# kivicode/TensorHive-Fixed

Measured on AMD Instinct MI355X. Metric: llama3_8b_bf16_ddp_train_tokens_per_sec, higher is better.
Workload: dtype bf16; 1 GPU; model=Llama-3-8B, global_batch=8, micro_batch=8, grad_accum=1, seq_len=4096, parallelism=dp1, optimizer=AdamW (fp32 master, fused flat kernel, clip 1.0), zero=0, attention=hip, gemm_table=True, gemm_table_kind=gemm_gfx950_t32768.csv

## Files before the change

tensorhive_fixed_amd/ops/csrc/cross_entropy.hip:

```cpp
#include "th_common.h"

__global__ __launch_bounds__(512) void ce_fwd_bwd_kernel(ushort* __restrict__ logits, long ld,
                                                         const long* __restrict__ target,
                                                         float* __restrict__ loss,
                                                         float* __restrict__ lse_out, int V,
                                                         float grad_scale, int ignore_index) {
  __shared__ float sm[16], ss[16];
  const long row = blockIdx.x;
  ushort* lr = logits + row * ld;
  const int nvec = (ld & 7) == 0 ? (V >> 3) : 0;
  float m = -INFINITY, s = 0.f;
  for (int i = threadIdx.x; i < nvec; i += blockDim.x) {
    const ushort8 x = reinterpret_cast<const ushort8*>(lr)[i];
    float vmax = -INFINITY;
    float f[8];
#pragma unroll
    for (int j = 0; j < 8; ++j) {
      f[j] = bf2f(x[j]);
      vmax = fmaxf(vmax, f[j]);
    }
    float vs = 0.f;
#pragma unroll
    for (int j = 0; j < 8; ++j) vs += __expf(f[j] - vmax);
    lse_merge(m, s, vmax, vs);
  }
  for (int i = (nvec << 3) + threadIdx.x; i < V; i += blockDim.x) lse_merge(m, s, bf2f(lr[i]), 1.f);
#pragma unroll
  for (int o = 32; o > 0; o >>= 1) {
    const float m2 = __shfl_xor(m, o, 64), s2 = __shfl_xor(s, o, 64);
    lse_merge(m, s, m2, s2);
  }
  const int lane = threadIdx.x & 63, wid = threadIdx.x >> 6;
  if (lane == 0) { sm[wid] = m; ss[wid] = s; }
  __syncthreads();
  m = sm[0]; s = ss[0];
  for (int w = 1; w < (int)(blockDim.x >> 6); ++w) lse_merge(m, s, sm[w], ss[w]);
  const float lse = m + __logf(s);
  const long tgt = target[row];
  const bool valid = tgt != ignore_index && tgt >= 0 && tgt < V;
  if (threadIdx.x == 0) {
    lse_out[row] = lse;
    loss[row] = valid ? (lse - bf2f(lr[tgt])) : 0.f;
  }
  __syncthreads();
  const float gs = valid ? grad_scale : 0.f;
  for (int i = threadIdx.x; i < nvec; i += blockDim.x) {
    const ushort8 x = reinterpret_cast<const ushort8*>(lr)[i];
    ushort8 o;
#pragma unroll
    for (int j = 0; j < 8; ++j) {
      float p = __expf(bf2f(x[j]) - lse);
      if (valid && (long)(i * 8 + j) == tgt) p -= 1.f;
      o[j] = f2bf(p * gs);
    }
    reinterpret_cast<ushort8*>(lr)[i] = o;
  }
  for (int i = (nvec << 3) + threadIdx.x; i < V; i += blockDim.x) {
    float p = __expf(bf2f(lr[i]) - lse);
    if (valid && (long)i == tgt) p -= 1.f;
    lr[i] = f2bf(p * gs);
  }
}

extern "C" int th_ce_fwd_bwd(void* logits, long ld, const long* target, float* loss, float* lse,
                             long rows, int V, float grad_scale, int ignore_index, hipStream_t s) {
  if (rows <= 0 || V <= 0 || ld < V) return -1;
  ce_fwd_bwd_kernel<<<(unsigned)rows, 512, 0, s>>>((ushort*)logits, ld, target, loss, lse, V,
                                                  grad_scale, ignore_index);
  TH_CHECK_LAUNCH();
}
```

tensorhive_fixed_amd/ops/csrc/rmsnorm.hip:

```cpp
#include "th_common.h"

template <int MAXV, bool ADD>
__global__ __launch_bounds__(256) void rmsnorm_fwd_kernel(const ushort* __restrict__ x,
                                                              const ushort* __restrict__ addend,
                                                              ushort* __restrict__ xsum,
                                                              const ushort* __restrict__ w,
                                                              ushort* __restrict__ y,
                                                              float* __restrict__ rstd_out, int D,
                                                              float eps) {
  __shared__ float red[16];
  const int row = blockIdx.x;
  const int nvec = D >> 3;
  const ushort8* xr = reinterpret_cast<const ushort8*>(x + (size_t)row * D);
  ushort8 cache[MAXV];
  float ss = 0.f;
#pragma unroll
  for (int i = 0; i < MAXV; ++i) {
    const int v = threadIdx.x + i * blockDim.x;
    if (v < nvec) {
      cache[i] = xr[v];
      if (ADD) {
        const ushort8 a = reinterpret_cast<const ushort8*>(addend + (size_t)row * D)[v];
#pragma unroll
        for (int j = 0; j < 8; ++j) cache[i][j] = f2bf(bf2f(cache[i][j]) + bf2f(a[j]));
        reinterpret_cast<ushort8*>(xsum + (size_t)row * D)[v] = cache[i];
      }
#pragma unroll
      for (int j = 0; j < 8; ++j) {
        const float f = bf2f(cache[i][j]);
        ss += f * f;
      }
    }
  }
  ss = block_sum(ss, red);
  const float r = rsqrtf(ss / (float)D + eps);
  if (threadIdx.x == 0) rstd_out[row] = r;
  const ushort8* wr = reinterpret_cast<const ushort8*>(w);
  ushort8* yr = reinterpret_cast<ushort8*>(y + (size_t)row * D);
#pragma unroll
  for (int i = 0; i < MAXV; ++i) {
    const int v = threadIdx.x + i * blockDim.x;
    if (v < nvec) {
      const ushort8 wv = wr[v];
      ushort8 o;
#pragma unroll
      for (int j = 0; j < 8; ++j) o[j] = f2bf(bf2f(cache[i][j]) * r * bf2f(wv[j]));
      yr[v] = o;
    }
  }
}

template <int MAXV>
__global__ __launch_bounds__(256) void rmsnorm_bwd_kernel(const ushort* __restrict__ dy,
                                                          const ushort* __restrict__ x,
                                                          const ushort* __restrict__ w,
                                                          const float* __restrict__ rstd,
                                                          ushort* __restrict__ dx,
                                                          float* __restrict__ ws, int T, int D,
                                                          const ushort* __restrict__ dres) {
  __shared__ float red[16];
  const int nvec = D >> 3;
  float dwacc[MAXV][8];
  float wreg[MAXV][8];
  const ushort8* wr = reinterpret_cast<const ushort8*>(w);
#pragma unroll
  for (int i = 0; i < MAXV; ++i) {
    const int v = threadIdx.x + i * blockDim.x;
    ushort8 wv = (v < nvec) ? wr[v] : ushort8(0);
#pragma unroll
    for (int j = 0; j < 8; ++j) {
      dwacc[i][j] = 0.f;
      wreg[i][j] = bf2f(wv[j]);
    }
  }
  for (int row = blockIdx.x; row < T; row += gridDim.x) {
    const ushort8* xr = reinterpret_cast<const ushort8*>(x + (size_t)row * D);
    const ushort8* gr = reinterpret_cast<const ushort8*>(dy + (size_t)row * D);
    ushort8 xc[MAXV], gc[MAXV], rc[MAXV];
    float dot = 0.f;
#pragma unroll
    for (int i = 0; i < MAXV; ++i) {
      const int v = threadIdx.x + i * blockDim.x;
      if (v < nvec) {
        xc[i] = xr[v];
        gc[i] = gr[v];
        rc[i] = dres ? reinterpret_cast<const ushort8*>(dres + (size_t)row * D)[v] : ushort8(0);
#pragma unroll
        for (int j = 0; j < 8; ++j) dot += bf2f(gc[i][j]) * wreg[i][j] * bf2f(xc[i][j]);
      }
    }
    dot = block_sum(dot, red);
    const float r = rstd[row];
    const float c = dot * r * r * r / (float)D;
    ushort8* dxr = reinterpret_cast<ushort8*>(dx + (size_t)row * D);
#pragma unroll
    for (int i = 0; i < MAXV; ++i) {
      const int v = threadIdx.x + i * blockDim.x;
      if (v < nvec) {
        ushort8 o;
#pragma unroll
        for (int j = 0; j < 8; ++j) {
          const float xf = bf2f(xc[i][j]), gf = bf2f(gc[i][j]);
          o[j] = f2bf(r * gf * wreg[i][j] - xf * c + bf2f(rc[i][j]));
          dwacc[i][j] += gf * xf * r;
        }
        dxr[v] = o;
      }
    }
  }
  float* wsr = ws + (size_t)blockIdx.x * D;
#pragma unroll
  for (int i = 0; i < MAXV; ++i) {
    const int v = threadIdx.x + i * blockDim.x;
    if (v < nvec) {
      float4v* p = reinterpret_cast<float4v*>(wsr + v * 8);
      p[0] = float4v{dwacc[i][0], dwacc[i][1], dwacc[i][2], dwacc[i][3]};
      p[1] = float4v{dwacc[i][4], dwacc[i][5], dwacc[i][6], dwacc[i][7]};
    }
  }
}

__global__ __launch_bounds__(256) void slab_reduce_bf16_kernel(const float* __restrict__ ws, ushort* __restrict__ out,
                                                               int nslab, int D, int accumulate) {
  __shared__ float4v part[16][16];
  const int cg = threadIdx.x & 15, sg = threadIdx.x >> 4;
  const int c = blockIdx.x * 64 + cg * 4;
  float4v acc = {0.f, 0.f, 0.f, 0.f};
  if (c < D) {
#pragma unroll 4
    for (int b = sg; b < nslab; b += 16) acc += *reinterpret_cast<const float4v*>(ws + (size_t)b * D + c);
  }
  part[sg][cg] = acc;
  __syncthreads();
  if (sg == 0 && c < D) {
    float4v t = part[0][cg];
#pragma unroll
    for (int k = 1; k < 16; ++k) t += part[k][cg];
#pragma unroll
    for (int j = 0; j < 4; ++j) {
      float v = t[j];
      if (accumulate) v += bf2f(out[c + j]);
      out[c + j] = f2bf(v);
    }
  }
}

static int pick_maxv(int D, int threads) { return (D / 8 + threads - 1) / threads; }

extern "C" int th_rmsnorm_fwd(const void* x, const void* w, void* y, float* rstd, int T, int D,
                              float eps, hipStream_t s) {
  if (D % 8 != 0 || T <= 0) return -1;
  const int mv = pick_maxv(D, 256);
  dim3 g(T), b(256);
  if (mv <= 2)
    rmsnorm_fwd_kernel<2, false><<<g, b, 0, s>>>((const ushort*)x, nullptr, nullptr, (const ushort*)w, (ushort*)y, rstd, D, eps);
  else if (mv <= 4)
    rmsnorm_fwd_kernel<4, false><<<g, b, 0, s>>>((const ushort*)x, nullptr, nullptr, (const ushort*)w, (ushort*)y, rstd, D, eps);
  else if (mv <= 8)
    rmsnorm_fwd_kernel<8, false><<<g, b, 0, s>>>((const ushort*)x, nullptr, nullptr, (const ushort*)w, (ushort*)y, rstd, D, eps);
  else
    return -2;
  TH_CHECK_LAUNCH();
}

extern "C" int th_rmsnorm_add_fwd(const void* x, const void* addend, const void* w, void* xsum, void* y,
                                  float* rstd, int T, int D, float eps, hipStream_t s) {
  if (D % 8 != 0 || T <= 0) return -1;
  const int mv = pick_maxv(D, 256);
  dim3 g(T), b(256);
#define TH_RMS_ADD(MV)                                                                                   \
  rmsnorm_fwd_kernel<MV, true><<<g, b, 0, s>>>((const ushort*)x, (const ushort*)addend, (ushort*)xsum, \
                                               (const ushort*)w, (ushort*)y, rstd, D, eps)
  if (mv <= 2)
    TH_RMS_ADD(2);
  else if (mv <= 4)
    TH_RMS_ADD(4);
  else if (mv <= 8)
    TH_RMS_ADD(8);
  else
    return -2;
#undef TH_RMS_ADD
  TH_CHECK_LAUNCH();
}

extern "C" int th_rmsnorm_bwd(const void* dy, const void* x, const void* w, const float* rstd,
                              void* dx, void* dw, float* ws, int nblk, int T, int D,
                              int accumulate, const void* dres, hipStream_t s) {
  if (D % 8 != 0 || T <= 0 || nblk <= 0) return -1;
  const int mv = pick_maxv(D, 256);
  dim3 g(nblk), b(256);
  if (mv <= 2)
    rmsnorm_bwd_kernel<2><<<g, b, 0, s>>>((const ushort*)dy, (const ushort*)x, (const ushort*)w, rstd, (ushort*)dx, ws, T, D, (const ushort*)dres);
  else if (mv <= 4)
    rmsnorm_bwd_kernel<4><<<g, b, 0, s>>>((const ushort*)dy, (const ushort*)x, (const ushort*)w, rstd, (ushort*)dx, ws, T, D, (const ushort*)dres);
  else if (mv <= 8)
    rmsnorm_bwd_kernel<8><<<g, b, 0, s>>>((const ushort*)dy, (const ushort*)x, (const ushort*)w, rstd, (ushort*)dx, ws, T, D, (const ushort*)dres);
  else
    return -2;
  slab_reduce_bf16_kernel<<<dim3((D + 63) / 64), dim3(256), 0, s>>>(ws, (ushort*)dw, nblk, D, accumulate);
  TH_CHECK_LAUNCH();
}
```

tensorhive_fixed_amd/ops/csrc/swiglu.hip:

```cpp
#include "th_common.h"

__device__ __forceinline__ float sigmoidf_(float g) { return 1.f / (1.f + __expf(-g)); }

__global__ __launch_bounds__(256) void swiglu_fwd_kernel(const ushort* __restrict__ gu,
                                                         ushort* __restrict__ out, long T, int F) {
  const int cpr = F >> 3;
  for (long row = blockIdx.x; row < T; row += gridDim.x) {
    const ushort* g_row = gu + row * 2 * F;
    ushort* o_row = out + row * F;
    for (int c = threadIdx.x; c < cpr; c += blockDim.x) {
      const ushort8 g = *reinterpret_cast<const ushort8*>(g_row + c * 8);
      const ushort8 u = *reinterpret_cast<const ushort8*>(g_row + F + c * 8);
      ushort8 o;
#pragma unroll
      for (int j = 0; j < 8; ++j) {
        const float gf = bf2f(g[j]);
        o[j] = f2bf(gf * sigmoidf_(gf) * bf2f(u[j]));
      }
      *reinterpret_cast<ushort8*>(o_row + c * 8) = o;
    }
  }
}

__global__ __launch_bounds__(256) void swiglu_bwd_kernel(const ushort* __restrict__ dout,
                                                         const ushort* __restrict__ gu,
                                                         ushort* __restrict__ dgu, long T, int F) {
  const int cpr = F >> 3;
  for (long row = blockIdx.x; row < T; row += gridDim.x) {
    for (int c = threadIdx.x; c < cpr; c += blockDim.x) {
      const ushort8 g = *reinterpret_cast<const ushort8*>(gu + row * 2 * F + c * 8);
      const ushort8 u = *reinterpret_cast<const ushort8*>(gu + row * 2 * F + F + c * 8);
      const ushort8 d = *reinterpret_cast<const ushort8*>(dout + row * F + c * 8);
      ushort8 dg, du;
#pragma unroll
      for (int j = 0; j < 8; ++j) {
        const float gf = bf2f(g[j]), uf = bf2f(u[j]), df = bf2f(d[j]);
        const float sg = sigmoidf_(gf);
        const float silu = gf * sg;
        du[j] = f2bf(df * silu);
        dg[j] = f2bf(df * uf * sg * (1.f + gf * (1.f - sg)));
      }
      *reinterpret_cast<ushort8*>(dgu + row * 2 * F + c * 8) = dg;
      *reinterpret_cast<ushort8*>(dgu + row * 2 * F + F + c * 8) = du;
    }
  }
}

constexpr int ST_R = 128, ST_C = 64;

__device__ __forceinline__ int st_swz(int r) { return 2 * (((r >> 1) & 1) | (((r >> 3) & 1) << 1)); }
__device__ __forceinline__ int st_off(int r, int chunk) { return r * 128 + ((chunk ^ st_swz(r)) << 4); }

typedef short i16x4s __attribute__((ext_vector_type(4)));
#define ST_LDS __attribute__((address_space(3)))

__global__ __launch_bounds__(256) void swiglu_bwd_t_kernel(const ushort* __restrict__ dout,
                                                           const ushort* __restrict__ gu,
                                                           ushort* __restrict__ dgu,
                                                           ushort* __restrict__ dguT, long T, int F) {
  __shared__ __attribute__((aligned(16))) char tile[2 * ST_R * 128];
  const int tid = threadIdx.x;
  const long ntc = F / ST_C;
  const long r0 = (blockIdx.x / ntc) * ST_R, c0 = (blockIdx.x % ntc) * ST_C;
  const int lch = tid & 7, lc = lch * 8;
  ushort8 g[4], u[4], d[4];
#pragma unroll
  for (int i = 0; i < 4; ++i) {
    const long row = r0 + (tid >> 3) + 32 * i;
    const long rr = row < T ? row : T - 1;
    g[i] = *reinterpret_cast<const ushort8*>(gu + rr * 2 * F + c0 + lc);
    u[i] = *reinterpret_cast<const ushort8*>(gu + rr * 2 * F + F + c0 + lc);
    d[i] = *reinterpret_cast<const ushort8*>(dout + rr * F + c0 + lc);
  }
#pragma unroll
  for (int i = 0; i < 4; ++i) {
    const int lr = (tid >> 3) + 32 * i;
    const long row = r0 + lr;
    ushort8 dg, du;
#pragma unroll
    for (int j = 0; j < 8; ++j) {
      const float gf = bf2f(g[i][j]), uf = bf2f(u[i][j]), df = bf2f(d[i][j]);
      const float sg = sigmoidf_(gf);
      du[j] = f2bf(df * gf * sg);
      dg[j] = f2bf(df * uf * sg * (1.f + gf * (1.f - sg)));
    }
    if (row < T) {
      *reinterpret_cast<ushort8*>(dgu + row * 2 * F + c0 + lc) = dg;
      *reinterpret_cast<ushort8*>(dgu + row * 2 * F + F + c0 + lc) = du;
    }
    *reinterpret_cast<ushort8*>(tile + st_off(lr, lch)) = dg;
    *reinterpret_cast<ushort8*>(tile + ST_R * 128 + st_off(lr, lch)) = du;
  }
  __syncthreads();
  const int lane = tid & 63, w = tid >> 6, grp = lane >> 4, i16 = lane & 15, q = i16 >> 2, p = i16 & 3;
#pragma unroll
  for (int k = 0; k < 8; ++k) {
    const int step = w * 8 + k;
    const int half = step >> 4, fb = (step >> 2) & 3, tg0 = (step & 3) * 32;
    const int rbase = tg0 + 8 * grp;
    const int col = fb * 16 + 4 * p;
    const char* base = tile + half * ST_R * 128 + ((col & 7) << 1);
    const int ch = col >> 3;
    const i16x4s lo = __builtin_amdgcn_ds_read_tr16_b64_v4i16((ST_LDS i16x4s*)(base + st_off(rbase + q, ch)));
    const i16x4s hi = __builtin_amdgcn_ds_read_tr16_b64_v4i16((ST_LDS i16x4s*)(base + st_off(rbase + 4 + q, ch)));
    ushort8 o;
#pragma unroll
    for (int e = 0; e < 4; ++e) {
      o[e] = (ushort)lo[e];
      o[4 + e] = (ushort)hi[e];
    }
    const long feat = (long)half * F + c0 + fb * 16 + i16;
    const long tok = r0 + rbase;
    if (tok < T) *reinterpret_cast<ushort8*>(dguT + feat * T + tok) = o;
  }
}

static unsigned grid_for(long rows) {
  long g = rows;
  if (g > 4096) g = 4096;
  if (g < 1) g = 1;
  return (unsigned)g;
}

extern "C" int th_swiglu_fwd(const void* gu, void* out, long T, int F, hipStream_t s) {
  if (F % 8 != 0 || T <= 0) return -1;
  swiglu_fwd_kernel<<<grid_for(T), 256, 0, s>>>((const ushort*)gu, (ushort*)out, T, F);
  TH_CHECK_LAUNCH();
}

extern "C" int th_swiglu_bwd(const void* dout, const void* gu, void* dgu, long T, int F,
                             hipStream_t s) {
  if (F % 8 != 0 || T <= 0) return -1;
  swiglu_bwd_kernel<<<grid_for(T), 256, 0, s>>>((const ushort*)dout, (const ushort*)gu,
                                                          (ushort*)dgu, T, F);
  TH_CHECK_LAUNCH();
}

extern "C" int th_swiglu_bwd_t(const void* dout, const void* gu, void* dgu, void* dguT, long T, int F,
                               hipStream_t s) {
  if (F % ST_C != 0 || T <= 0 || T % 8 != 0) return -1;
  const long tiles = ((T + ST_R - 1) / ST_R) * (F / ST_C);
  if (tiles > 0x7fffffffL) return -2;
  swiglu_bwd_t_kernel<<<(unsigned)tiles, 256, 0, s>>>((const ushort*)dout, (const ushort*)gu, (ushort*)dgu,
                                                      (ushort*)dguT, T, F);
  TH_CHECK_LAUNCH();
}
```

tensorhive_fixed_amd/ops/csrc/transpose.hip:

```cpp
#include "th_common.h"

template <int TR, int TC>
__global__ __launch_bounds__(256) void transpose_bf16_kernel(const ushort* __restrict__ in,
                                                             ushort* __restrict__ out, long R, long C,
                                                             long ld_in) {
  constexpr int PITCH = TC + 2;
  constexpr int LPR = TC / 8;
  constexpr int RPP = 256 / LPR;
  constexpr int OPL = 256 / TC;
  constexpr int RPL = TR / OPL;
  __shared__ ushort tile[TR * PITCH];
  const int tid = threadIdx.x;
  const long ntc = (C + TC - 1) / TC;
  const long bt = blockIdx.x;
  const long r0 = (bt / ntc) * TR, c0 = (bt % ntc) * TC;

  const int lc = (tid % LPR) * 8;
  ushort8 v[TR / RPP];
#pragma unroll
  for (int i = 0; i < TR / RPP; ++i) {
    const int lr = tid / LPR + RPP * i;
    v[i] = ushort8(0);
    if (r0 + lr < R && c0 + lc < C) v[i] = *reinterpret_cast<const ushort8*>(in + (r0 + lr) * ld_in + c0 + lc);
  }
#pragma unroll
  for (int i = 0; i < TR / RPP; ++i) {
    const int lr = tid / LPR + RPP * i;
    unsigned* dst = reinterpret_cast<unsigned*>(tile + lr * PITCH + lc);
#pragma unroll
    for (int j = 0; j < 4; ++j) dst[j] = (unsigned)v[i][2 * j] | ((unsigned)v[i][2 * j + 1] << 16);
  }
  __syncthreads();

  const int oc = tid / OPL;
  const int orr = (tid % OPL) * RPL;
  if (c0 + oc >= C) return;
  ushort* orow = out + (c0 + oc) * R + r0 + orr;
#pragma unroll
  for (int q = 0; q < RPL / 8; ++q) {
    ushort8 w;
#pragma unroll
    for (int j = 0; j < 8; ++j) w[j] = tile[(orr + 8 * q + j) * PITCH + oc];
    if (r0 + orr + 8 * q < R) *reinterpret_cast<ushort8*>(orow + 8 * q) = w;
  }
}

extern "C" int th_transpose_bf16(const void* in, void* out, long R, long C, long ld_in, int tile, hipStream_t s) {
  if (R <= 0 || C <= 0 || R % 8 || C % 8 || ld_in % 8 || ld_in < C) return -1;
  auto launch = [&](auto kern, long tr, long tc) {
    const long tiles = ((R + tr - 1) / tr) * ((C + tc - 1) / tc);
    if (tiles > 0x7fffffffL) return -2;
    kern<<<(unsigned)tiles, 256, 0, s>>>((const ushort*)in, (ushort*)out, R, C, ld_in);
    return (int)hipGetLastError();
  };
  if (tile == 0) tile = C > 16384 ? 1 : 3;
  switch (tile) {
    case 2: return launch(transpose_bf16_kernel<128, 128>, 128, 128);
    case 3: return launch(transpose_bf16_kernel<64, 128>, 64, 128);
    default: return launch(transpose_bf16_kernel<128, 64>, 128, 64);
  }
}
```

Before: 27020 tokens/s.

## Batch loads in CE, SwiGLU, RMSNorm bwd and use LDS transpose reads

The cross-entropy kernel now keeps the whole logits row in registers, so the gradient pass no longer reloads it from memory. RMSNorm backward prefetches the next row's inputs while the current row is computed. SwiGLU kernels batch eight vector loads per thread and use nontemporal loads and stores. The transpose kernel switches to a swizzled LDS layout read with ds_read_tr16_b64 transposing loads. Together these aim to cut memory traffic and latency stalls, at the cost of higher register pressure and lower occupancy.

```diff
diff --git a/tensorhive_fixed_amd/ops/csrc/cross_entropy.hip b/tensorhive_fixed_amd/ops/csrc/cross_entropy.hip
--- a/tensorhive_fixed_amd/ops/csrc/cross_entropy.hip
+++ b/tensorhive_fixed_amd/ops/csrc/cross_entropy.hip
@@ -1,5 +1,8 @@
 #include "th_common.h"
 
+constexpr int CE_SLOTS = 32;
+
+template <bool HOLD>
 __global__ __launch_bounds__(512) void ce_fwd_bwd_kernel(ushort* __restrict__ logits, long ld,
                                                          const long* __restrict__ target,
                                                          float* __restrict__ loss,
@@ -10,8 +13,8 @@
   ushort* lr = logits + row * ld;
   const int nvec = (ld & 7) == 0 ? (V >> 3) : 0;
   float m = -INFINITY, s = 0.f;
-  for (int i = threadIdx.x; i < nvec; i += blockDim.x) {
-    const ushort8 x = reinterpret_cast<const ushort8*>(lr)[i];
+  ushort8 held[HOLD ? CE_SLOTS : 1];
+  auto merge_vec = [&](const ushort8 x) {
     float vmax = -INFINITY;
     float f[8];
 #pragma unroll
@@ -23,6 +26,18 @@
 #pragma unroll
     for (int j = 0; j < 8; ++j) vs += __expf(f[j] - vmax);
     lse_merge(m, s, vmax, vs);
+  };
+  if (HOLD) {
+#pragma unroll
+    for (int k = 0; k < CE_SLOTS; ++k) {
+      const int i = threadIdx.x + k * 512;
+      if (i < nvec) held[k] = reinterpret_cast<const ushort8*>(lr)[i];
+    }
+#pragma unroll
+    for (int k = 0; k < CE_SLOTS; ++k)
+      if ((int)threadIdx.x + k * 512 < nvec) merge_vec(held[k]);
+  } else {
+    for (int i = threadIdx.x; i < nvec; i += blockDim.x) merge_vec(reinterpret_cast<const ushort8*>(lr)[i]);
   }
   for (int i = (nvec << 3) + threadIdx.x; i < V; i += blockDim.x) lse_merge(m, s, bf2f(lr[i]), 1.f);
 #pragma unroll
@@ -44,8 +59,7 @@
   }
   __syncthreads();
   const float gs = valid ? grad_scale : 0.f;
-  for (int i = threadIdx.x; i < nvec; i += blockDim.x) {
-    const ushort8 x = reinterpret_cast<const ushort8*>(lr)[i];
+  auto grad_vec = [&](const ushort8 x, int i) {
     ushort8 o;
 #pragma unroll
     for (int j = 0; j < 8; ++j) {
@@ -54,6 +68,15 @@
       o[j] = f2bf(p * gs);
     }
     reinterpret_cast<ushort8*>(lr)[i] = o;
+  };
+  if (HOLD) {
+#pragma unroll
+    for (int k = 0; k < CE_SLOTS; ++k) {
+      const int i = threadIdx.x + k * 512;
+      if (i < nvec) grad_vec(held[k], i);
+    }
+  } else {
+    for (int i = threadIdx.x; i < nvec; i += blockDim.x) grad_vec(reinterpret_cast<const ushort8*>(lr)[i], i);
   }
   for (int i = (nvec << 3) + threadIdx.x; i < V; i += blockDim.x) {
     float p = __expf(bf2f(lr[i]) - lse);
@@ -65,7 +88,12 @@
 extern "C" int th_ce_fwd_bwd(void* logits, long ld, const long* target, float* loss, float* lse,
                              long rows, int V, float grad_scale, int ignore_index, hipStream_t s) {
   if (rows <= 0 || V <= 0 || ld < V) return -1;
-  ce_fwd_bwd_kernel<<<(unsigned)rows, 512, 0, s>>>((ushort*)logits, ld, target, loss, lse, V,
-                                                  grad_scale, ignore_index);
+  const bool hold = (ld & 7) == 0 && ((uintptr_t)logits & 15) == 0 && (V >> 3) <= 512 * CE_SLOTS;
+  if (hold)
+    ce_fwd_bwd_kernel<true><<<(unsigned)rows, 512, 0, s>>>((ushort*)logits, ld, target, loss, lse, V,
+                                                          grad_scale, ignore_index);
+  else
+    ce_fwd_bwd_kernel<false><<<(unsigned)rows, 512, 0, s>>>((ushort*)logits, ld, target, loss, lse, V,
+                                                           grad_scale, ignore_index);
   TH_CHECK_LAUNCH();
 }
diff --git a/tensorhive_fixed_amd/ops/csrc/rmsnorm.hip b/tensorhive_fixed_amd/ops/csrc/rmsnorm.hip
--- a/tensorhive_fixed_amd/ops/csrc/rmsnorm.hip
+++ b/tensorhive_fixed_amd/ops/csrc/rmsnorm.hip
@@ -73,24 +73,39 @@
       wreg[i][j] = bf2f(wv[j]);
     }
   }
-  for (int row = blockIdx.x; row < T; row += gridDim.x) {
+  ushort8 xc[MAXV], gc[MAXV], rc[MAXV];
+  float rcur = 0.f;
+  auto load_row = [&](int row, ushort8(&xo)[MAXV], ushort8(&go)[MAXV], ushort8(&ro)[MAXV], float& rs) {
     const ushort8* xr = reinterpret_cast<const ushort8*>(x + (size_t)row * D);
     const ushort8* gr = reinterpret_cast<const ushort8*>(dy + (size_t)row * D);
-    ushort8 xc[MAXV], gc[MAXV], rc[MAXV];
-    float dot = 0.f;
 #pragma unroll
     for (int i = 0; i < MAXV; ++i) {
       const int v = threadIdx.x + i * blockDim.x;
       if (v < nvec) {
-        xc[i] = xr[v];
-        gc[i] = gr[v];
-        rc[i] = dres ? reinterpret_cast<const ushort8*>(dres + (size_t)row * D)[v] : ushort8(0);
+        xo[i] = xr[v];
+        go[i] = gr[v];
+        ro[i] = dres ? reinterpret_cast<const ushort8*>(dres + (size_t)row * D)[v] : ushort8(0);
+      }
+    }
+    rs = rstd[row];
+  };
+  if ((int)blockIdx.x < T) load_row(blockIdx.x, xc, gc, rc, rcur);
+  for (int row = blockIdx.x; row < T; row += gridDim.x) {
+    ushort8 xn[MAXV], gn[MAXV], rn[MAXV];
+    float rnext = 0.f;
+    const int nrow = row + gridDim.x;
+    if (nrow < T) load_row(nrow, xn, gn, rn, rnext);
+    float dot = 0.f;
+#pragma unroll
+    for (int i = 0; i < MAXV; ++i) {
+      const int v = threadIdx.x + i * blockDim.x;
+      if (v < nvec) {
 #pragma unroll
         for (int j = 0; j < 8; ++j) dot += bf2f(gc[i][j]) * wreg[i][j] * bf2f(xc[i][j]);
       }
     }
     dot = block_sum(dot, red);
-    const float r = rstd[row];
+    const float r = rcur;
     const float c = dot * r * r * r / (float)D;
     ushort8* dxr = reinterpret_cast<ushort8*>(dx + (size_t)row * D);
 #pragma unroll
@@ -107,6 +122,13 @@
         dxr[v] = o;
       }
     }
+#pragma unroll
+    for (int i = 0; i < MAXV; ++i) {
+      xc[i] = xn[i];
+      gc[i] = gn[i];
+      rc[i] = rn[i];
+    }
+    rcur = rnext;
   }
   float* wsr = ws + (size_t)blockIdx.x * D;
 #pragma unroll
diff --git a/tensorhive_fixed_amd/ops/csrc/swiglu.hip b/tensorhive_fixed_amd/ops/csrc/swiglu.hip
--- a/tensorhive_fixed_amd/ops/csrc/swiglu.hip
+++ b/tensorhive_fixed_amd/ops/csrc/swiglu.hip
@@ -1,6 +1,16 @@
 #include "th_common.h"
 
 __device__ __forceinline__ float sigmoidf_(float g) { return 1.f / (1.f + __expf(-g)); }
+
+constexpr int SW_BATCH = 8;
+
+__device__ __forceinline__ ushort8 sw_load(const ushort* p) { return *reinterpret_cast<const ushort8*>(p); }
+__device__ __forceinline__ ushort8 sw_load_nt(const ushort* p) {
+  return __builtin_nontemporal_load(reinterpret_cast<const ushort8*>(p));
+}
+__device__ __forceinline__ void sw_store_nt(ushort* p, ushort8 v) {
+  __builtin_nontemporal_store(v, reinterpret_cast<ushort8*>(p));
+}
 
 __global__ __launch_bounds__(256) void swiglu_fwd_kernel(const ushort* __restrict__ gu,
                                                          ushort* __restrict__ out, long T, int F) {
@@ -8,16 +18,29 @@
   for (long row = blockIdx.x; row < T; row += gridDim.x) {
     const ushort* g_row = gu + row * 2 * F;
     ushort* o_row = out + row * F;
-    for (int c = threadIdx.x; c < cpr; c += blockDim.x) {
-      const ushort8 g = *reinterpret_cast<const ushort8*>(g_row + c * 8);
-      const ushort8 u = *reinterpret_cast<const ushort8*>(g_row + F + c * 8);
-      ushort8 o;
+    for (int c0 = threadIdx.x; c0 < cpr; c0 += SW_BATCH * 256) {
+      ushort8 g[SW_BATCH], u[SW_BATCH];
 #pragma unroll
-      for (int j = 0; j < 8; ++j) {
-        const float gf = bf2f(g[j]);
-        o[j] = f2bf(gf * sigmoidf_(gf) * bf2f(u[j]));
+      for (int k = 0; k < SW_BATCH; ++k) {
+        const int c = c0 + k * 256;
+        if (c < cpr) {
+          g[k] = sw_load(g_row + c * 8);
+          u[k] = sw_load(g_row + F + c * 8);
+        }
       }
-      *reinterpret_cast<ushort8*>(o_row + c * 8) = o;
+#pragma unroll
+      for (int k = 0; k < SW_BATCH; ++k) {
+        const int c = c0 + k * 256;
+        if (c < cpr) {
+          ushort8 o;
+#pragma unroll
+          for (int j = 0; j < 8; ++j) {
+            const float gf = bf2f(g[k][j]);
+            o[j] = f2bf(gf * sigmoidf_(gf) * bf2f(u[k][j]));
+          }
+          sw_store_nt(o_row + c * 8, o);
+        }
+      }
     }
   }
 }
@@ -27,21 +50,37 @@
                                                          ushort* __restrict__ dgu, long T, int F) {
   const int cpr = F >> 3;
   for (long row = blockIdx.x; row < T; row += gridDim.x) {
-    for (int c = threadIdx.x; c < cpr; c += blockDim.x) {
-      const ushort8 g = *reinterpret_cast<const ushort8*>(gu + row * 2 * F + c * 8);
-      const ushort8 u = *reinterpret_cast<const ushort8*>(gu + row * 2 * F + F + c * 8);
-      const ushort8 d = *reinterpret_cast<const ushort8*>(dout + row * F + c * 8);
-      ushort8 dg, du;
+    const ushort* g_row = gu + row * 2 * F;
+    const ushort* d_row = dout + row * F;
+    ushort* o_row = dgu + row * 2 * F;
+    for (int c0 = threadIdx.x; c0 < cpr; c0 += SW_BATCH * 256) {
+      ushort8 g[SW_BATCH], u[SW_BATCH], d[SW_BATCH];
 #pragma unroll
-      for (int j = 0; j < 8; ++j) {
-        const float gf = bf2f(g[j]), uf = bf2f(u[j]), df = bf2f(d[j]);
-        const float sg = sigmoidf_(gf);
-        const float silu = gf * sg;
-        du[j] = f2bf(df * silu);
-        dg[j] = f2bf(df * uf * sg * (1.f + gf * (1.f - sg)));
+      for (int k = 0; k < SW_BATCH; ++k) {
+        const int c = c0 + k * 256;
+        if (c < cpr) {
+          g[k] = sw_load_nt(g_row + c * 8);
+          u[k] = sw_load_nt(g_row + F + c * 8);
+          d[k] = sw_load(d_row + c * 8);
+        }
       }
-      *reinterpret_cast<ushort8*>(dgu + row * 2 * F + c * 8) = dg;
-      *reinterpret_cast<ushort8*>(dgu + row * 2 * F + F + c * 8) = du;
+#pragma unroll
+      for (int k = 0; k < SW_BATCH; ++k) {
+        const int c = c0 + k * 256;
+        if (c < cpr) {
+          ushort8 dg, du;
+#pragma unroll
+          for (int j = 0; j < 8; ++j) {
+            const float gf = bf2f(g[k][j]), uf = bf2f(u[k][j]), df = bf2f(d[k][j]);
+            const float sg = sigmoidf_(gf);
+            const float silu = gf * sg;
+            du[j] = f2bf(df * silu);
+            dg[j] = f2bf(df * uf * sg * (1.f + gf * (1.f - sg)));
+          }
+          sw_store_nt(o_row + c * 8, dg);
+          sw_store_nt(o_row + F + c * 8, du);
+        }
+      }
     }
   }
 }
diff --git a/tensorhive_fixed_amd/ops/csrc/transpose.hip b/tensorhive_fixed_amd/ops/csrc/transpose.hip
--- a/tensorhive_fixed_amd/ops/csrc/transpose.hip
+++ b/tensorhive_fixed_amd/ops/csrc/transpose.hip
@@ -1,21 +1,27 @@
 #include "th_common.h"
+
+__device__ __forceinline__ int tp_swz(int r) { return 2 * (((r >> 1) & 1) | (((r >> 3) & 1) << 1)); }
+__device__ __forceinline__ int tp_off(int r, int chunk) { return r * 128 + ((chunk ^ tp_swz(r)) << 4); }
+
+typedef short tp_i16x4 __attribute__((ext_vector_type(4)));
+#define TP_LDS __attribute__((address_space(3)))
 
 template <int TR, int TC>
 __global__ __launch_bounds__(256) void transpose_bf16_kernel(const ushort* __restrict__ in,
                                                              ushort* __restrict__ out, long R, long C,
                                                              long ld_in) {
-  constexpr int PITCH = TC + 2;
   constexpr int LPR = TC / 8;
   constexpr int RPP = 256 / LPR;
-  constexpr int OPL = 256 / TC;
-  constexpr int RPL = TR / OPL;
-  __shared__ ushort tile[TR * PITCH];
+  constexpr int IMG = TR * 128;
+  constexpr int TGS = TR / 32;
+  constexpr int SPW = (TC / 16) * TGS / 4;
+  __shared__ __attribute__((aligned(16))) char tile[TR * TC * 2];
   const int tid = threadIdx.x;
   const long ntc = (C + TC - 1) / TC;
   const long bt = blockIdx.x;
   const long r0 = (bt / ntc) * TR, c0 = (bt % ntc) * TC;
 
-  const int lc = (tid % LPR) * 8;
+  const int lch = tid % LPR, lc = lch * 8;
   ushort8 v[TR / RPP];
 #pragma unroll
   for (int i = 0; i < TR / RPP; ++i) {
@@ -26,22 +32,29 @@
 #pragma unroll
   for (int i = 0; i < TR / RPP; ++i) {
     const int lr = tid / LPR + RPP * i;
-    unsigned* dst = reinterpret_cast<unsigned*>(tile + lr * PITCH + lc);
-#pragma unroll
-    for (int j = 0; j < 4; ++j) dst[j] = (unsigned)v[i][2 * j] | ((unsigned)v[i][2 * j + 1] << 16);
+    *reinterpret_cast<ushort8*>(tile + (lch >> 3) * IMG + tp_off(lr, lch & 7)) = v[i];
   }
   __syncthreads();
 
-  const int oc = tid / OPL;
-  const int orr = (tid % OPL) * RPL;
-  if (c0 + oc >= C) return;
-  ushort* orow = out + (c0 + oc) * R + r0 + orr;
+  const int lane = tid & 63, w = tid >> 6, grp = lane >> 4, i16 = lane & 15, q = i16 >> 2, p = i16 & 3;
 #pragma unroll
-  for (int q = 0; q < RPL / 8; ++q) {
-    ushort8 w;
+  for (int k = 0; k < SPW; ++k) {
+    const int step = w * SPW + k;
+    const int fb = step / TGS, tg0 = (step % TGS) * 32;
+    const int rbase = tg0 + 8 * grp;
+    const int col = fb * 16 + 4 * p;
+    const char* base = tile + (col >> 6) * IMG + ((col & 7) << 1);
+    const int ch = (col & 63) >> 3;
+    const tp_i16x4 lo = __builtin_amdgcn_ds_read_tr16_b64_v4i16((TP_LDS tp_i16x4*)(base + tp_off(rbase + q, ch)));
+    const tp_i16x4 hi = __builtin_amdgcn_ds_read_tr16_b64_v4i16((TP_LDS tp_i16x4*)(base + tp_off(rbase + 4 + q, ch)));
+    ushort8 o;
 #pragma unroll
-    for (int j = 0; j < 8; ++j) w[j] = tile[(orr + 8 * q + j) * PITCH + oc];
-    if (r0 + orr + 8 * q < R) *reinterpret_cast<ushort8*>(orow + 8 * q) = w;
+    for (int e = 0; e < 4; ++e) {
+      o[e] = (ushort)lo[e];
+      o[4 + e] = (ushort)hi[e];
+    }
+    const long oc = c0 + fb * 16 + i16, orow = r0 + rbase;
+    if (oc < C && orow < R) *reinterpret_cast<ushort8*>(out + oc * R + orow) = o;
   }
 }
 
```

New measurement: 27070 tokens/s, median of 6. Within noise of the previous version (+0.2%).
